# ModelCloud/GPTQModel

Measured on NVIDIA B200. Metric: W4A16 g128 QuantLinear: decode tok/s + prefill TFLOPS vs HBM/TC roofline, higher is better.
Workload: dtype f16

## Files before the change

gptqmodel_b200/_lib.py:

```python
from __future__ import annotations

import ctypes
import os

_HERE = os.path.dirname(os.path.abspath(__file__))
LIB_PATH = os.path.join(_HERE, "libb2q.so")

ABI_VERSION = 3

_vp, _i, _sz = ctypes.c_void_p, ctypes.c_int, ctypes.c_size_t
SYMBOLS = {
    "b2q_version": (_i, []),
    "b2q_last_error": (ctypes.c_char_p, []),
    "b2q_packed_bytes": (_sz, [_i, _i, _i]),
    "b2q_workspace_bytes": (_sz, [_i, _i, _i, _i]),
    "b2q_mm_workspace_bytes": (_sz, [_i, _i, _i, _i, _i, _i]),
    "b2q_debug_reload_env": (None, []),
    "b2q_prepack": (_i, [_vp, _vp, _vp, _i, _i, _i, _vp]),
    "b2q_mm": (_i, [_vp, _vp, _vp, _vp, _vp, _vp, _vp, _i, _i, _i, _i, _i, _i, _vp, _sz, _vp]),
    "b2q_decode": (_i, [_vp, _vp, _vp, _vp, _vp, _vp, _vp, _i, _i, _i, _i, _i, _i, _i, _i, _vp]),
    "b2q_decode_multi": (_i, [_vp, _i, _vp, _vp, _vp, _vp, _vp, _vp, _vp, _i, _i, _i, _i, _i, _vp]),
    "b2q_gemm_multi": (_i, [_vp, _i, _vp, _vp, _vp, _vp, _vp, _vp, _vp, _i, _i, _i, _i, _i, _vp, _sz, _vp]),
    "b2q_gemv": (_i, [_vp, _vp, _vp, _vp, _vp, _vp, _vp, _i, _i, _i, _i, _i, _i, _i, _vp]),
    "b2q_gemm": (_i, [_vp, _vp, _vp, _vp, _vp, _vp, _vp, _i, _i, _i, _i, _i, _i, _vp, _sz, _vp]),
    "b2q_allreduce": (_i, [_vp, _i, _i, _i, _i, _vp, _sz, _i, _vp, _vp]),
    "b2q_decode_allreduce": (_i, [_vp, _vp, _vp, _vp, _vp, _vp, _i, _i, _i, _i, _i, _i, _i, _i, _vp, _sz, _i, _vp, _vp]),
    "b2q_decode_allreduce_flag_bytes": (_sz, []),
    "b2q_debug_set_trace": (None, [_vp]),
    "b2q_debug_decode_plan": (_i, [_i, _i, _i, _i, _i, _i, _vp]),
    "b2q_permute_cols": (_i, [_vp, _vp, _vp, _i, _i, _vp]),
    "b2q_moe_align": (_i, [_vp, _i, _i, _i, _vp, _vp, _vp, _vp]),
    "b2q_moe_gather": (_i, [_vp, _vp, _vp, _i, _i, _i, _vp]),
    "b2q_moe_gate_up": (_i, [_vp, _vp, _vp, _vp, _vp, _vp, _vp, _vp, _vp, _vp, _i, _i, _i, _i, _i, _i, _i, _i, _vp]),
    "b2q_moe_down": (_i, [_vp, _vp, _vp, _vp, _vp, _vp, _vp, _vp, _vp, _i, _i, _i, _i, _i, _i, _i, _i, _vp]),
    "b2q_moe_combine": (_i, [_vp, _vp, _i, _i, _i, _i, _vp]),
    "b2q_moe_decode_gate_up": (_i, [_vp, _vp, _vp, _vp, _vp, _vp, _vp, _vp, _i, _i, _i, _i, _i, _i, _i, _vp, _vp]),
# ... 33 lines not shown
```

gptqmodel_b200/csrc/b2q_api.cu:

```cuda
#include <cstdarg>
#include <cstdio>
#include <cstdlib>

#include "../../include/b2q.h"
#include "b2q_internal.h"

namespace b2q {
static thread_local char g_err[512] = "";

void set_error(const char* fmt, ...) {
  va_list ap;
  va_start(ap, fmt);
  vsnprintf(g_err, sizeof(g_err), fmt, ap);
  va_end(ap);
}

static int env_int(const char* name, int dflt) {
  const char* e = getenv(name);
  return (e != nullptr && e[0] != 0) ? atoi(e) : dflt;
}

static EnvCfg read_env() {
  EnvCfg c;
  c.disable_pdl = env_int("B2Q_DISABLE_PDL", 0);
  c.gemm_1cta = env_int("B2Q_GEMM_1CTA", 0);
  c.midm = env_int("B2Q_MIDM", 1);
  c.decode_blocks_m = env_int("B2Q_DECODE_BLOCKS_M", 0);
  c.decode_groups2 = env_int("B2Q_DECODE_GROUPS", 1) == 2;
  c.decode_v2 = env_int("B2Q_DECODE_V2", -1);
  c.decode2_gw = env_int("B2Q_DECODE2_GW", 0);
  c.decode2_ks = env_int("B2Q_DECODE2_KS", 0);
  c.decode2_xtma = env_int("B2Q_DECODE2_XTMA", 0);
  c.decode2_fastsync = env_int("B2Q_DECODE2_FASTSYNC", 0);
  c.gemm2_persist = env_int("B2Q_GEMM2_PERSIST", 1);
  c.gemm2_dqw = env_int("B2Q_GEMM2_DQW", 8) == 4 ? 4 : 8;
  c.midm_ks = env_int("B2Q_MIDM_KS", 0);
  c.midm_dqg1 = env_int("B2Q_MIDM_DQG1", 0);
  return c;
}

static EnvCfg g_env = read_env();
const EnvCfg& env() { return g_env; }
void reload_env() { g_env = read_env(); }

struct DeviceGuard {
  int prev = -1, dev = -1;
  explicit DeviceGuard(const void* p) {
    cudaPointerAttributes at;
    if (p != nullptr && cudaPointerGetAttributes(&at, p) == cudaSuccess && at.type == cudaMemoryTypeDevice) {
      dev = at.device;
      if (cudaGetDevice(&prev) == cudaSuccess && prev != dev) cudaSetDevice(dev);
      else prev = -1;
    }
    (void)cudaGetLastError();
  }
  ~DeviceGuard() {
    if (prev >= 0) cudaSetDevice(prev);
  }
};

static int check_cuda(int e, const char* what) {
  if (e > 0) set_error("%s: CUDA error %d (%s)", what, e, cudaGetErrorString((cudaError_t)e));
  return e;
}

static int validate(const char* fn, const void* x, const void* packed, const void* scales, const void* out, int M,
                    int K, int N, int bits, int group_size, int dtype) {
  if (x == nullptr || packed == nullptr || scales == nullptr || out == nullptr) {
    set_error("%s: null pointer argument", fn);
    return -2;
  }
  if (bits != 4 && bits != 8) {
    set_error("%s: bits=%d not supported (4 or 8)", fn, bits);
    return -2;
  }
  if (dtype != B2Q_DTYPE_F16 && dtype != B2Q_DTYPE_BF16) {
    set_error("%s: dtype=%d not supported (0 fp16, 1 bf16)", fn, dtype);
    return -2;
// ... 25 lines not shown
  a.perm = perm;
  a.bias = bias;
  a.out = out;
  a.M = M;
  a.K = K;
  a.N = N;
  a.bits = bits;
  a.group_size = group_size;
  a.dtype = dtype;
  a.workspace = workspace;
  a.workspace_bytes = workspace_bytes;
  a.stream = (cudaStream_t)stream;
  a.tune_ks = 0;
  a.tune_warps = 0;
  a.pdl = env().disable_pdl ? 0 : 1;
  return a;
}
}

using namespace b2q;

extern "C" {

int b2q_version(void) { return B2Q_ABI_VERSION; }

void b2q_debug_set_trace(void* device_buffer) { g_trace_ptr = device_buffer; }

int b2q_debug_decode_plan(int version, int M, int K, int N, int ks, int warps, int* out8) {
  if (out8 == nullptr || (version != 1 && version != 2) || M < 1 || M > 8 || K < 128 || K % 128 != 0 || N < 32 ||
      N % 32 != 0) {
// ... 155 lines not shown
  MmArgs a = make_args(x, packed, scales, qzeros, perm, bias, out, M, K, N, bits, group_size, dtype, nullptr, 0,
                       stream);
  a.tune_ks = ks;
  a.tune_warps = warps;
  if (!decode_supported(a)) {
    set_error("b2q_decode: needs bits=4, 1 <= M <= 8, K %% 128 == 0, group_size 64|128|K (got bits=%d M=%d K=%d g=%d)",
              bits, M, K, group_size);
    return -2;
  }
  return check_cuda(launch_decode(a), "b2q_decode");
}

int b2q_decode_multi(const void* x, int nsets, const void* const* packed, const void* const* scales,
                     const int32_t* const* qzeros, const int32_t* perm, const void* const* bias, void* const* out,
                     const int* N, int M, int K, int bits, int group_size, int dtype, void* stream) {
  if (x == nullptr || packed == nullptr || scales == nullptr || qzeros == nullptr || bias == nullptr ||
      out == nullptr || N == nullptr || nsets < 1) {
    set_error("b2q_decode_multi: null pointer argument");
    return -2;
  }
  int v = validate("b2q_decode_multi", x, packed[0], scales[0], out[0], M, K, N[0], bits, group_size, dtype);
  if (v != 0) return v;
  DeviceGuard dg(packed[0]);
  MmArgs a = make_args(x, packed[0], scales[0], qzeros[0], perm, bias[0], out[0], M, K, N[0], bits, group_size,
                       dtype, nullptr, 0, stream);
  return check_cuda(launch_decode_multi(a, nsets, packed, scales, qzeros, bias, out, N), "b2q_decode_multi");
}

int b2q_gemm_multi(const void* x, int nsets, const void* const* packed, const void* const* scales,
                   const int32_t* const* qzeros, const int32_t* perm, const void* const* bias, void* const* out,
                   const int* N, int M, int K, int bits, int group_size, int dtype, void* workspace,
                   size_t workspace_bytes, void* stream) {
  if (x == nullptr || packed == nullptr || scales == nullptr || qzeros == nullptr || bias == nullptr ||
      out == nullptr || N == nullptr || nsets < 1) {
    set_error("b2q_gemm_multi: null pointer argument");
    return -2;
  }
  int v = validate("b2q_gemm_multi", x, packed[0], scales[0], out[0], M, K, N[0], bits, group_size, dtype);
  if (v != 0) return v;
  if (bits != 4 || M <= 128) {
// ... 21 lines not shown
             const void* bias, void* out, int M, int K, int N, int bits, int group_size, int dtype, void* workspace,
             size_t workspace_bytes, void* stream) {
  int v = validate("b2q_gemm", x, packed, scales, out, M, K, N, bits, group_size, dtype);
  if (v != 0) return v;
  DeviceGuard dg(packed);
  if (M == 0) return 0;
  MmArgs a = make_args(x, packed, scales, qzeros, perm, bias, out, M, K, N, bits, group_size, dtype, workspace,
                       workspace_bytes, stream);
  if (env().gemm_1cta) a.tune_ks = -1;
  return check_cuda(launch_gemm(a), "b2q_gemm");
}

int b2q_mm(const void* x, const void* packed, const void* scales, const int32_t* qzeros, const int32_t* perm,
           const void* bias, void* out, int M, int K, int N, int bits, int group_size, int dtype, void* workspace,
           size_t workspace_bytes, void* stream) {
  int v = validate("b2q_mm", x, packed, scales, out, M, K, N, bits, group_size, dtype);
  if (v != 0) return v;
  DeviceGuard dg(packed);
  if (M == 0) return 0;
  MmArgs a = make_args(x, packed, scales, qzeros, perm, bias, out, M, K, N, bits, group_size, dtype, workspace,
                       workspace_bytes, stream);
  if (decode_supported(a)) return check_cuda(launch_decode(a), "b2q_mm(decode)");
  {
    MmArgs a8 = a;
    a8.M = 8;
    if (M > 8 && M <= env().decode_blocks_m && decode_supported(a8) && perm == nullptr) {
      for (int m0 = 0; m0 < M; m0 += 8) {
        MmArgs ab = a;
        ab.M = (M - m0 < 8) ? (M - m0) : 8;
        ab.x = static_cast<const char*>(x) + (size_t)m0 * K * 2;
        ab.out = static_cast<char*>(out) + (size_t)m0 * N * 2;
        int e = check_cuda(launch_decode(ab), "b2q_mm(decode x blocks)");
        if (e != 0) return e;
      }
      return 0;
    }
  }
// ... 141 lines not shown
```

gptqmodel_b200/csrc/b2q_decode.cu:

```cuda
#include "b2q_common.cuh"
#include "b2q_decode.cuh"
#include "b2q_internal.h"

namespace b2q {

template <typename T, bool ASYM, bool G64, bool MOE>
__global__ void __launch_bounds__(DEC_MAX_WARPS * 32)
    decode_kernel(const __grid_constant__ DecSets S, const int32_t* __restrict__ perm, const T* __restrict__ x, int M,
                  int K, int gsh, int qpc, int max_tiles, int ngroups, int stl,
                  const __grid_constant__ DecodeAR ar, unsigned long long* __restrict__ trace) {
  using E = ET<T>;
  extern __shared__ __align__(128) uint8_t dsm[];
  auto stamp = [&](int slot) {
    if (trace != nullptr && threadIdx.x == 0 && blockIdx.y == 0) {
      unsigned long long tns;
      asm volatile("mov.u64 %0, %%globaltimer;" : "=l"(tns));
      trace[blockIdx.x * 16 + slot] = tns;
    }
  };
  stamp(0);
  if (MOE) asm volatile("griddepcontrol.wait;" ::: "memory");
  const int lane = threadIdx.x & 31, warp = threadIdx.x >> 5, nwarps = blockDim.x >> 5;
  const int g = lane >> 2, t = lane & 3;
  const int gw = nwarps / ngroups;
  const int grp = warp / gw, wg = warp - grp * gw;
// ... 32 lines not shown
      iss_q = 0;
      ++iss_ti;
      if (iss_u < U) iss_begin_tile();
    } else {
      iss_src += (size_t)(2 * gw) * iss_kbs;
    }
  };
  if (lane == 0) {
#pragma unroll
    for (int i = 0; i < DEC_STAGES; ++i) mbar_init(bars + 8 * i, 1);
    fence_mbar_init();
    if (U > 0) iss_begin_tile();
#pragma unroll
    for (int i = 0; i < DEC_STAGES; ++i)
      if (i < nst && iss_u < U) iss_one(smem_u32(ring) + i * DEC_QUAD_BYTES, bars + 8 * i);
  }
  const int gstep = (2 * gw) >> gsh;
  const int g_first = (2 * (q0 + wg)) >> gsh;
  const T* sc_next = nullptr;
  const uint32_t* zq_next = nullptr;
  int pre_q = 0, pre_ti = 0, pre_N = 0;
  auto pre_begin_tile = [&]() {
    const TileRef<T> r = resolve_tile<T, MOE>(S, tile0 + pre_ti * C);
    pre_N = r.N;
    sc_next = r.sc + (size_t)g_first * r.N + r.nt * 32 + g;
    if (ASYM) zq_next = r.zq + (size_t)g_first * (r.N >> 3) + r.nt * 4;
  };
  auto fetch_scales = [&](DScale<ASYM, G64>& d) {
#pragma unroll
    for (int i = 0; i < 4; ++i) {
// ... 157 lines not shown
              zh = (float)((cur.zw[ASYM ? gi : 0][ftl * 2 + 1] >> (4 * g)) & 15u);
            }
            const float bl = E::LO_BASE + zl, bh = E::HI_BASE + zh;
            float d[4];
#pragma unroll
            for (int c = 0; c < 4; ++c) d[c] = G64 ? dd[kbl][ftl][c] : dd[0][ftl][c] + dd[1][ftl][c];
            tot[ftl][0] = fmaf(sl, d[0] - bl * xs0, tot[ftl][0]);
            tot[ftl][1] = fmaf(sl, d[1] - bl * xs1, tot[ftl][1]);
            tot[ftl][2] = fmaf(sh, d[2] * E::HI_SCALE - bh * xs0, tot[ftl][2]);
            tot[ftl][3] = fmaf(sh, d[3] * E::HI_SCALE - bh * xs1, tot[ftl][3]);
          }
          xs0 = xs1 = 0.f;
        }
      }
      __syncwarp();
      if (lane == 0 && iss_u < U) iss_one(ring_a + st * DEC_QUAD_BYTES, bars + 8 * st);
      if (u + 1 < U) cur = nxt;
    }

    if (ti < 5) stamp(4 + 2 * ti);
    float* rbuf = red + (grp * 2 + (ti & 1)) * gw * 256;
#pragma unroll
    for (int a = 0; a < 2; ++a)
#pragma unroll
      for (int b = 0; b < 4; ++b) rbuf[(wg * 8 + a * 4 + b) * 32 + lane] = tot[a][b];
    asm volatile("bar.sync %0, %1;" ::"r"(1 + grp), "r"(gw * 32) : "memory");
    for (int i = wg * 32 + lane; i < 256; i += gw * 32) {
      float v = 0.f;
      for (int w = 0; w < gw; ++w) v += rbuf[w * 256 + i];
      if (nrank > 1) {
        part[(grp * max_tiles + ti) * 256 + i] = v;
// ... 76 lines not shown
            if (MOE && S.moe >= 2) pr = S.wts[r] * E::to_f(E::from_f(pr));
            v += pr;
          }
          const int n = nt * 32 + (acc >> 2) * 16 + (ln >> 2) + ((acc & 2) ? 8 : 0);
          T o = E::from_f(v);
          if (bias != nullptr) o = E::from_f(E::to_f(o) + E::to_f(bias[n]));
          out[(size_t)m * N + n] = o;
        }
      }
    }
    cluster_sync_all();
  }
}

void* g_trace_ptr = nullptr;

struct DecodeCfg {
  int C, ks, warps, qpc, max_tiles, ngroups, stl;
  size_t smem;
};

static size_t decode_smem(int M, int warps, int qpc, int max_tiles, int nst) {
  return (size_t)warps * nst * DEC_QUAD_BYTES + (size_t)M * qpc * 128 * 2 + (size_t)qpc * 2 * 8 * 4 +
         (size_t)2 * warps * 256 * 4 + (size_t)max_tiles * 256 * 4 + (size_t)warps * DEC_STAGES * 8 + 16;
}

static bool decode_config(const MmArgs& a, int NT, DecodeCfg& best) {
  const int quads = a.K / 128;
  const int SMS = 148;
  double best_cost = 1e30;
// ... 55 lines not shown
  cfg.blockDim = dim3(c.warps * 32, 1, 1);
  cfg.dynamicSmemBytes = c.smem;
  cfg.stream = a.stream;
  cudaLaunchAttribute attr[2];
  attr[0].id = cudaLaunchAttributeClusterDimension;
  attr[0].val.clusterDim.x = 1;
  attr[0].val.clusterDim.y = c.ks;
  attr[0].val.clusterDim.z = 1;
  attr[1].id = cudaLaunchAttributeProgrammaticStreamSerialization;
  attr[1].val.programmaticStreamSerializationAllowed = 1;
  cfg.attrs = attr;
  cfg.numAttrs = a.pdl ? 2 : 1;
  int gsh = 31;
  if (a.group_size == 64) gsh = 0;
  else if (a.group_size == 128) gsh = 1;
  cudaError_t e = cudaLaunchKernelEx(&cfg, kern, sets, a.perm, (const T*)a.x, a.M, a.K, gsh, c.qpc, c.max_tiles,
                                     c.ngroups, c.stl, ar, (unsigned long long*)g_trace_ptr);
  return (int)e;
}

bool decode_supported(const MmArgs& a) {
  return a.bits == 4 && a.M >= 1 && a.M <= DEC_MAXM && a.K % 128 == 0 && a.N % 32 == 0 &&
         (a.group_size == 64 || a.group_size == 128 || a.group_size == a.K);
}

int launch_decode2_sets(const MmArgs& a, const DecSets& sets);

static int launch_decode_sets(const MmArgs& a, const DecSets& sets) {
  {
    const int mode = env().decode_v2;
    const int NT = sets.tile_end[sets.nsets - 1];
    if (mode == 1 || (mode < 0 && NT > 148 && a.tune_ks <= 0 && a.tune_warps <= 0)) {
// ... 187 lines not shown
```

gptqmodel_b200/csrc/b2q_decode.cuh:

```cuda
#pragma once
#include "b2q_common.cuh"

namespace b2q {

constexpr int DEC_MAX_WARPS = 16;
constexpr int DEC_MAXM = 8;

template <typename T>
__device__ __forceinline__ void mma_16816(float (&d)[4], const uint32_t (&a)[4], uint32_t b0, uint32_t b1);
template <>
__device__ __forceinline__ void mma_16816<__half>(float (&d)[4], const uint32_t (&a)[4], uint32_t b0, uint32_t b1) {
  asm volatile("mma.sync.aligned.m16n8k16.row.col.f32.f16.f16.f32 {%0,%1,%2,%3}, {%4,%5,%6,%7}, {%8,%9}, {%0,%1,%2,%3};"
               : "+f"(d[0]), "+f"(d[1]), "+f"(d[2]), "+f"(d[3])
               : "r"(a[0]), "r"(a[1]), "r"(a[2]), "r"(a[3]), "r"(b0), "r"(b1));
}
template <>
__device__ __forceinline__ void mma_16816<__nv_bfloat16>(float (&d)[4], const uint32_t (&a)[4], uint32_t b0,
                                                         uint32_t b1) {
  asm volatile(
      "mma.sync.aligned.m16n8k16.row.col.f32.bf16.bf16.f32 {%0,%1,%2,%3}, {%4,%5,%6,%7}, {%8,%9}, {%0,%1,%2,%3};"
      : "+f"(d[0]), "+f"(d[1]), "+f"(d[2]), "+f"(d[3])
      : "r"(a[0]), "r"(a[1]), "r"(a[2]), "r"(a[3]), "r"(b0), "r"(b1));
}

// ... 180 lines not shown
  int nsets;
  int tile_end[DEC_MAX_SETS];
  int N[DEC_MAX_SETS];
  const uint4* packed[DEC_MAX_SETS];
  const void* scales[DEC_MAX_SETS];
  const uint32_t* qzeros[DEC_MAX_SETS];
  const void* bias[DEC_MAX_SETS];
  void* out[DEC_MAX_SETS];
  int moe;
  int nexperts;
  const int32_t* ids;
  const float* wts;
  size_t estride_w, estride_s, estride_z;
};

template <typename T>
struct TileRef {
  const uint4* w;
  const T* sc;
  const uint32_t* zq;
  const T* bias;
  T* out;
  int N, nt;
};

template <typename T, bool MOE = false>
__device__ __forceinline__ TileRef<T> resolve_tile(const DecSets& S, int gt) {
  TileRef<T> r;
  if (MOE) {
    int s = 0, nt = gt, slot;
// ... 41 lines not shown
```

gptqmodel_b200/csrc/b2q_decode2.cu:

```cuda
#include "b2q_common.cuh"
#include "b2q_decode.cuh"
#include "b2q_internal.h"

namespace b2q {

constexpr int DEC_AR_MAXCTA = 160;
int launch_decode1_allreduce(const MmArgs& a, const DecSets& sets, const DecodeAR& ar);

__device__ __forceinline__ void cluster_sync_cta_fenced() {
  asm volatile("fence.acq_rel.cta;\n\tbarrier.cluster.arrive.relaxed.aligned;\n\tbarrier.cluster.wait.aligned;" ::: "memory");
}

__device__ __forceinline__ void dec_st_release_sys(uint32_t* p, uint32_t v) {
  asm volatile("st.release.sys.global.u32 [%0], %1;" ::"l"(p), "r"(v) : "memory");
}
__device__ __forceinline__ uint32_t dec_ld_acquire_sys(const uint32_t* p) {
  uint32_t v;
  asm volatile("ld.acquire.sys.global.u32 %0, [%1];" : "=r"(v) : "l"(p) : "memory");
  return v;
}

template <typename T, bool ASYM, bool G64, bool MOE>
__global__ void __launch_bounds__(DEC_MAX_WARPS * 32)
    decode2_kernel(const __grid_constant__ DecSets S, const int32_t* __restrict__ perm, const T* __restrict__ x, int M,
                   int K, int gsh, int qpc, int max_tiles, int gw, int stl, int xtma,
                   const __grid_constant__ DecodeAR ar, unsigned long long* __restrict__ trace) {
  using E = ET<T>;
  extern __shared__ __align__(128) uint8_t dsm2[];
  auto stamp = [&](int slot) {
    if (trace != nullptr && threadIdx.x == 0 && blockIdx.y == 0) {
      unsigned long long tns;
      asm volatile("mov.u64 %0, %%globaltimer;" : "=l"(tns));
      trace[blockIdx.x * 16 + slot] = tns;
    }
  };
  stamp(0);
  if (MOE) asm volatile("griddepcontrol.wait;" ::: "memory");
  const int lane = threadIdx.x & 31, warp = threadIdx.x >> 5, nwarps = blockDim.x >> 5;
  const int g = lane >> 2, t = lane & 3;
  const int ngroups = nwarps / gw;
  const int grp = warp / gw, wg = warp - grp * gw;
// ... 37 lines not shown
      ++iss_ti;
      if (iss_u < U) iss_begin_tile();
    } else {
      iss_src += (size_t)(2 * gw) * iss_kbs;
    }
  };
  if (lane == 0) {
#pragma unroll
    for (int i = 0; i < DEC_STAGES; ++i) mbar_init(bars + 8 * i, 1);
    if (warp == 0) mbar_init(xbar, 1);
    fence_mbar_init();
    if (U > 0) iss_begin_tile();
#pragma unroll
    for (int i = 0; i < DEC_STAGES; ++i)
      if (i < nst && iss_u < U) iss_one(smem_u32(ring) + i * DEC_QUAD_BYTES, bars + 8 * i);
  }
  const int gstep = (2 * gw) >> gsh;
  const int g_first = (2 * (q0 + wg)) >> gsh;
  const T* sc_next = nullptr;
  const uint32_t* zq_next = nullptr;
  int pre_q = 0, pre_ti = 0, pre_N = 0;
  auto pre_begin_tile = [&]() {
    const TileRef<T> r = resolve_tile<T, MOE>(S, tile0 + pre_ti * C);
    pre_N = r.N;
    sc_next = r.sc + (size_t)g_first * r.N + r.nt * 32 + g;
    if (ASYM) zq_next = r.zq + (size_t)g_first * (r.N >> 3) + r.nt * 4;
  };
  auto fetch_scales = [&](DScale<ASYM, G64>& d) {
#pragma unroll
    for (int i = 0; i < 4; ++i) {
// ... 165 lines not shown
              zh = (float)((cur.zw[ASYM ? gi : 0][ftl * 2 + 1] >> (4 * g)) & 15u);
            }
            const float bl = E::LO_BASE + zl, bh = E::HI_BASE + zh;
            float d[4];
#pragma unroll
            for (int c = 0; c < 4; ++c) d[c] = G64 ? dd[kbl][ftl][c] : dd[0][ftl][c] + dd[1][ftl][c];
            tot[ftl][0] = fmaf(sl, d[0] - bl * xs0, tot[ftl][0]);
            tot[ftl][1] = fmaf(sl, d[1] - bl * xs1, tot[ftl][1]);
            tot[ftl][2] = fmaf(sh, d[2] * E::HI_SCALE - bh * xs0, tot[ftl][2]);
            tot[ftl][3] = fmaf(sh, d[3] * E::HI_SCALE - bh * xs1, tot[ftl][3]);
          }
          xs0 = xs1 = 0.f;
        }
      }
      __syncwarp();
      if (lane == 0 && iss_u < U) iss_one(ring_a + st * DEC_QUAD_BYTES, bars + 8 * st);
      if (u + 1 < U) cur = nxt;
    }

    float* wp = wpart + ((size_t)(grp * max_tiles + ti) * M * gw + wg) * 32;
#pragma unroll
    for (int a = 0; a < 2; ++a)
#pragma unroll
      for (int b = 0; b < 4; ++b) {
        const int m = 2 * t + (b & 1);
        if (m < M) {
          const int f = a * 16 + g + ((b & 2) ? 8 : 0);
          wp[(size_t)m * gw * 32 + ((f + 8 * t) & 31)] = tot[a][b];
        }
      }
  }
// ... 173 lines not shown
  cfg.dynamicSmemBytes = c.smem;
  cfg.stream = a.stream;
  cudaLaunchAttribute attr[2];
  attr[0].id = cudaLaunchAttributeClusterDimension;
  attr[0].val.clusterDim.x = 1;
  attr[0].val.clusterDim.y = c.ks;
  attr[0].val.clusterDim.z = 1;
  attr[1].id = cudaLaunchAttributeProgrammaticStreamSerialization;
  attr[1].val.programmaticStreamSerializationAllowed = 1;
  cfg.attrs = attr;
  cfg.numAttrs = a.pdl ? 2 : 1;
  int gsh = 31;
  if (a.group_size == 64) gsh = 0;
  else if (a.group_size == 128) gsh = 1;
  const int xtma = (env().decode2_xtma ? 1 : 0) | (env().decode2_fastsync ? 2 : 0);
  cudaError_t e = cudaLaunchKernelEx(&cfg, kern, sets, a.perm, (const T*)a.x, a.M, a.K, gsh, c.qpc, c.max_tiles, c.gw,
                                     c.stl, xtma, ar, (unsigned long long*)g_trace_ptr);
  return (int)e;
}

static int launch_decode2_ar(const MmArgs& a, const DecSets& sets, const DecodeAR& ar) {
  Decode2Cfg c;
  if (!decode2_config(a, sets.tile_end[sets.nsets - 1], c)) return -2;
  if (ar.world > 1 && c.C * c.ks > DEC_AR_MAXCTA) return -2;
  const bool asym = a.qzeros != nullptr, g64 = a.group_size == 64;
#define B2Q_DEC2_CASE(T, MOE)                                                          \
  (asym ? (g64 ? launch_decode2_t<T, true, true, MOE>(a, sets, c, ar)                      \
               : launch_decode2_t<T, true, false, MOE>(a, sets, c, ar))                    \
        : (g64 ? launch_decode2_t<T, false, true, MOE>(a, sets, c, ar)                     \
               : launch_decode2_t<T, false, false, MOE>(a, sets, c, ar)))
  if (sets.moe != 0) return a.dtype == 0 ? B2Q_DEC2_CASE(__half, true) : B2Q_DEC2_CASE(__nv_bfloat16, true);
  return a.dtype == 0 ? B2Q_DEC2_CASE(__half, false) : B2Q_DEC2_CASE(__nv_bfloat16, false);
// ... 35 lines not shown
```

gptqmodel_b200/csrc/b2q_internal.h:

```cpp
#pragma once
#include <cuda_runtime.h>
#include <stdint.h>

namespace b2q {

struct MmArgs {
  const void* x;
  const void* packed;
  const void* scales;
  const void* qzeros;
  const int32_t* perm;
  const void* bias;
  void* out;
  int M, K, N;
  int bits;
  int group_size;
  int dtype;
  void* workspace;
  size_t workspace_bytes;
  cudaStream_t stream;
  int tune_ks;
  int tune_warps;
  int pdl;
};

struct DecodeAR {
  int world, rank;
  int max_elems;
  size_t flag_offset;
  void* buf[8];
  uint32_t* ctl;
};
int launch_decode_allreduce(const MmArgs& a, const DecodeAR& ar);
size_t decode_allreduce_flag_bytes();

int launch_prepack(const void* qweight, const int32_t* perm, void* out, int K, int N, int bits, cudaStream_t stream);
int launch_permute_cols(const void* x, const int32_t* perm, void* out, int M, int K, cudaStream_t stream);
int launch_gemv(const MmArgs& a);
// ... 39 lines not shown
struct EnvCfg {
  int disable_pdl;
  int gemm_1cta;
  int midm;
  int decode_blocks_m;
  int decode_groups2;
  int decode_v2;
  int decode2_gw;
  int decode2_ks;
  int decode2_xtma;
  int decode2_fastsync;
  int gemm2_persist;
  int gemm2_dqw;
  int midm_ks;
  int midm_dqg1;
};
const EnvCfg& env();
void reload_env();

template <typename Kern>
inline int ensure_dyn_smem(Kern kern, int bytes, uint32_t& done_mask, const char* who) {
  int dev = 0;
  cudaGetDevice(&dev);
  if (dev < 32 && ((done_mask >> dev) & 1u)) return 0;
  cudaError_t e = cudaFuncSetAttribute(kern, cudaFuncAttributeMaxDynamicSharedMemorySize, bytes);
  if (e != cudaSuccess) {
    set_error("%s: cannot opt in to %d bytes of shared memory: %s", who, bytes, cudaGetErrorString(e));
    return (int)e;
  }
  if (dev < 32) done_mask |= 1u << dev;
// ... 6 lines not shown
```

gptqmodel_b200/qlinear.py:

```python
from __future__ import annotations

import os

import math
from typing import Optional, Tuple

import torch
import torch.nn as nn

import ctypes

from . import layouts
from ._lib import B2QError, check, lib
from .adapter import Lora

_DTYPE_CODE = {torch.float16: 0, torch.bfloat16: 1}
DECODE_MAX_M = 8
PREFILL_MIN_M = 128


class SiblingGroup:

    def __init__(self, members):
        self.members = list(members)
        self.key = None
        self.pending = {}
        self._x_ref = None

    @staticmethod
    def _version(t):
        try:
            return t._version
        except RuntimeError:
# ... 8 lines not shown
                self._x_ref = None
            return out
        mods = self.members
        n = len(mods)
        K = who.in_features
        outs = [torch.empty((M, m.out_features), dtype=x2.dtype, device=x2.device) for m in mods]
        vp = ctypes.c_void_p * n
        packed = vp(*[m.packed.data_ptr() for m in mods])
        scales = vp(*[m._scales_for(x2.dtype).data_ptr() for m in mods])
        zeros = vp(*[_ptr(m._zeros_dev) for m in mods])
        bias = vp(*[_ptr(m._bias_for(x2.dtype)) for m in mods])
        outp = vp(*[o.data_ptr() for o in outs])
        Ns = (ctypes.c_int * n)(*[m.out_features for m in mods])
        stream = torch.cuda.current_stream(x2.device).cuda_stream
        if M <= DECODE_MAX_M:
            check(lib.b2q_decode_multi(x2.data_ptr(), n, packed, scales, zeros, _ptr(who.perm), bias, outp, Ns, M, K,
                                       who.kbits, who._kgs, _DTYPE_CODE[x2.dtype], stream), "b2q_decode_multi")
        else:
            ws, ws_bytes = None, 0
            if who.perm is not None:
                ws_bytes = M * K * 2
                ws = torch.empty(ws_bytes, dtype=torch.uint8, device=x2.device)
            check(lib.b2q_gemm_multi(x2.data_ptr(), n, packed, scales, zeros, _ptr(who.perm), bias, outp, Ns, M, K,
                                     who.kbits, who._kgs, _DTYPE_CODE[x2.dtype], _ptr(ws), ws_bytes, stream),
                  "b2q_gemm_multi")
        self.key = key
        self._x_ref = x2
        self.pending = {id(m): o for m, o in zip(mods, outs) if m is not who}
        return outs[mods.index(who)]


def fuse_siblings(mods) -> bool:
# ... 229 lines not shown
            x2 = x2.contiguous()
        M = x2.shape[0]
        if self._siblings is not None and (1 <= M <= DECODE_MAX_M or M > PREFILL_MIN_M):
            return self._siblings.run(self, x2, M).reshape(out_shape)
        out = torch.empty((M, N), dtype=x.dtype, device=x.device)
        if M == 0:
            return out.reshape(out_shape)
        if self._gather is not None:
            x2 = x2.index_select(1, self._gather)
        kK = self._kK
        ws, ws_bytes = None, 0
        if self.perm is not None:
            ws_bytes = lib.b2q_mm_workspace_bytes(M, kK, N, self.kbits, self._kgs, 1)
            if ws_bytes:
                ws = torch.empty(ws_bytes, dtype=torch.uint8, device=x.device)
        check(
            lib.b2q_mm(_ptr(x2), _ptr(self.packed), _ptr(self._scales_for(x.dtype)), _ptr(self._zeros_dev),
                       _ptr(self.perm), _ptr(self._bias_for(x.dtype)), _ptr(out), M, kK, N, self.kbits,
                       self._kgs, _DTYPE_CODE[x.dtype], _ptr(ws), ws_bytes,
                       torch.cuda.current_stream(x.device).cuda_stream),
            "b2q_mm",
        )
        out = out.reshape(out_shape)
        if self.adapter:
            out = self.adapter.apply(x=x, out=out)
        return out

    def forward_allreduce(self, x: torch.Tensor, ar) -> torch.Tensor:
        if not self._prepacked:
            raise B2QError("B200QuantLinear.forward_allreduce() before post_init()")
        K, N = self.in_features, self.out_features
        x2 = x.reshape(-1, K)
        if not x2.is_contiguous():
            x2 = x2.contiguous()
        M = x2.shape[0]
# ... 144 lines not shown
```

include/b2q.h:

```cpp
#ifndef B2Q_H_
#define B2Q_H_

#include <stddef.h>
#include <stdint.h>

#ifdef __cplusplus
extern "C" {
#endif

#define B2Q_ABI_VERSION 3
#define B2Q_DTYPE_F16 0
#define B2Q_DTYPE_BF16 1

int b2q_version(void);

const char* b2q_last_error(void);

size_t b2q_packed_bytes(int K, int N, int bits);

size_t b2q_workspace_bytes(int M, int K, int N, int has_perm);
size_t b2q_mm_workspace_bytes(int M, int K, int N, int bits, int group_size, int has_perm);

int b2q_prepack(const int32_t* qweight, const int32_t* perm, void* packed, int K, int N, int bits, void* stream);

int b2q_mm(const void* x, const void* packed, const void* scales, const int32_t* qzeros, const int32_t* perm,
           const void* bias, void* out, int M, int K, int N, int bits, int group_size, int dtype, void* workspace,
           size_t workspace_bytes, void* stream);

int b2q_decode(const void* x, const void* packed, const void* scales, const int32_t* qzeros, const int32_t* perm,
               const void* bias, void* out, int M, int K, int N, int bits, int group_size, int dtype, int ks,
               int warps, void* stream);
int b2q_gemv(const void* x, const void* packed, const void* scales, const int32_t* qzeros, const int32_t* perm,
             const void* bias, void* out, int K, int N, int bits, int group_size, int dtype, int ks, int warps,
             void* stream);
int b2q_gemm(const void* x, const void* packed, const void* scales, const int32_t* qzeros, const int32_t* perm,
             const void* bias, void* out, int M, int K, int N, int bits, int group_size, int dtype, void* workspace,
             size_t workspace_bytes, void* stream);

int b2q_decode_multi(const void* x, int nsets, const void* const* packed, const void* const* scales,
                     const int32_t* const* qzeros, const int32_t* perm, const void* const* bias, void* const* out,
                     const int* N, int M, int K, int bits, int group_size, int dtype, void* stream);

int b2q_gemm_multi(const void* x, int nsets, const void* const* packed, const void* const* scales,
                   const int32_t* const* qzeros, const int32_t* perm, const void* const* bias, void* const* out,
                   const int* N, int M, int K, int bits, int group_size, int dtype, void* workspace,
                   size_t workspace_bytes, void* stream);

int b2q_moe_align(const int32_t* topk_ids, int T, int top_k, int E, int32_t* counts, int32_t* offsets,
                  int32_t* sorted_pairs, void* stream);
int b2q_moe_gather(const void* x, const int32_t* sorted_pairs, void* xs, int rows, int top_k, int K, void* stream);
int b2q_moe_gate_up(const void* xs, const void* packed1, const void* scales1, const int32_t* qzeros1,
                    const void* packed3, const void* scales3, const int32_t* qzeros3, void* h, const int32_t* counts,
                    const int32_t* offsets, int E, int rows, int active, int K, int N, int bits, int group_size, int dtype,
                    void* stream);
int b2q_moe_down(const void* h, const void* packed2, const void* scales2, const int32_t* qzeros2, const int32_t* counts,
                 const int32_t* offsets, const int32_t* sorted_pairs, const float* pair_weights, float* ypair, int E,
// ... 33 lines not shown
```

Baseline: 866.9.

## Prefetch successor layer's weights into L2 during decode kernel tail

Records the order in which decode launchers run and passes a hint describing the next layer's packed weights, scales, zeros and perm into the decode kernel. Once a CTA has issued its last weight load, its warps issue cp.async.bulk.prefetch.L2 for the first tiles of the successor layer, capped by a configurable byte budget. The aim is to hide the next kernel's cold HBM ramp-up behind the current kernel's tail. In exchange it adds extra HBM traffic that competes with the current kernel's bandwidth, can pull in data that is never used if the recorded successor is wrong, and changes the ABI.

```diff
diff --git a/gptqmodel_b200/_lib.py b/gptqmodel_b200/_lib.py
--- a/gptqmodel_b200/_lib.py
+++ b/gptqmodel_b200/_lib.py
@@ -6,9 +6,24 @@
 _HERE = os.path.dirname(os.path.abspath(__file__))
 LIB_PATH = os.path.join(_HERE, "libb2q.so")
 
-ABI_VERSION = 3
+ABI_VERSION = 4
+
+HINT_MAX_SETS = 3
+
+
+class PrefetchHint(ctypes.Structure):
+    _fields_ = [
+        ("nsets", ctypes.c_int), ("K", ctypes.c_int), ("group_size", ctypes.c_int),
+        ("N", ctypes.c_int * HINT_MAX_SETS),
+        ("packed", ctypes.c_void_p * HINT_MAX_SETS),
+        ("scales", ctypes.c_void_p * HINT_MAX_SETS),
+        ("qzeros", ctypes.c_void_p * HINT_MAX_SETS),
+        ("perm", ctypes.c_void_p),
+    ]
+
 
 _vp, _i, _sz = ctypes.c_void_p, ctypes.c_int, ctypes.c_size_t
+_hint = ctypes.POINTER(PrefetchHint)
 SYMBOLS = {
     "b2q_version": (_i, []),
     "b2q_last_error": (ctypes.c_char_p, []),
@@ -20,6 +35,8 @@
     "b2q_mm": (_i, [_vp, _vp, _vp, _vp, _vp, _vp, _vp, _i, _i, _i, _i, _i, _i, _vp, _sz, _vp]),
     "b2q_decode": (_i, [_vp, _vp, _vp, _vp, _vp, _vp, _vp, _i, _i, _i, _i, _i, _i, _i, _i, _vp]),
     "b2q_decode_multi": (_i, [_vp, _i, _vp, _vp, _vp, _vp, _vp, _vp, _vp, _i, _i, _i, _i, _i, _vp]),
+    "b2q_mm_hinted": (_i, [_vp, _vp, _vp, _vp, _vp, _vp, _vp, _i, _i, _i, _i, _i, _i, _vp, _sz, _vp, _hint]),
+    "b2q_decode_multi_hinted": (_i, [_vp, _i, _vp, _vp, _vp, _vp, _vp, _vp, _vp, _i, _i, _i, _i, _i, _vp, _hint]),
     "b2q_gemm_multi": (_i, [_vp, _i, _vp, _vp, _vp, _vp, _vp, _vp, _vp, _i, _i, _i, _i, _i, _vp, _sz, _vp]),
     "b2q_gemv": (_i, [_vp, _vp, _vp, _vp, _vp, _vp, _vp, _i, _i, _i, _i, _i, _i, _i, _vp]),
     "b2q_gemm": (_i, [_vp, _vp, _vp, _vp, _vp, _vp, _vp, _i, _i, _i, _i, _i, _i, _vp, _sz, _vp]),
diff --git a/gptqmodel_b200/csrc/b2q_api.cu b/gptqmodel_b200/csrc/b2q_api.cu
--- a/gptqmodel_b200/csrc/b2q_api.cu
+++ b/gptqmodel_b200/csrc/b2q_api.cu
@@ -36,6 +36,7 @@
   c.gemm2_dqw = env_int("B2Q_GEMM2_DQW", 8) == 4 ? 4 : 8;
   c.midm_ks = env_int("B2Q_MIDM_KS", 0);
   c.midm_dqg1 = env_int("B2Q_MIDM_DQG1", 0);
+  c.xprefetch_bytes = env_int("B2Q_XPREFETCH_BYTES", 8 << 20);
   return c;
 }
 
@@ -62,6 +63,19 @@
 static int check_cuda(int e, const char* what) {
   if (e > 0) set_error("%s: CUDA error %d (%s)", what, e, cudaGetErrorString((cudaError_t)e));
   return e;
+}
+
+static int validate_hint(const char* fn, const b2q_prefetch_hint* h) {
+  if (h == nullptr || h->nsets == 0) return 0;
+  bool ok = h->nsets > 0 && h->nsets <= B2Q_HINT_MAX_SETS && h->K > 0 && h->K % 64 == 0 && h->group_size > 0 &&
+            h->K % h->group_size == 0;
+  for (int i = 0; ok && i < h->nsets; ++i)
+    ok = h->packed[i] != nullptr && h->scales[i] != nullptr && h->N[i] > 0 && h->N[i] % 32 == 0;
+  if (!ok) {
+    set_error("%s: malformed prefetch hint (nsets=%d K=%d group_size=%d)", fn, h->nsets, h->K, h->group_size);
+    return -2;
+  }
+  return 0;
 }
 
 static int validate(const char* fn, const void* x, const void* packed, const void* scales, const void* out, int M,
@@ -117,6 +131,7 @@
   a.tune_ks = 0;
   a.tune_warps = 0;
   a.pdl = env().disable_pdl ? 0 : 1;
+  a.hint = nullptr;
   return a;
 }
 }
@@ -302,16 +317,26 @@
 int b2q_decode_multi(const void* x, int nsets, const void* const* packed, const void* const* scales,
                      const int32_t* const* qzeros, const int32_t* perm, const void* const* bias, void* const* out,
                      const int* N, int M, int K, int bits, int group_size, int dtype, void* stream) {
+  return b2q_decode_multi_hinted(x, nsets, packed, scales, qzeros, perm, bias, out, N, M, K, bits, group_size, dtype,
+                                 stream, nullptr);
+}
+
+int b2q_decode_multi_hinted(const void* x, int nsets, const void* const* packed, const void* const* scales,
+                            const int32_t* const* qzeros, const int32_t* perm, const void* const* bias, void* const* out,
+                            const int* N, int M, int K, int bits, int group_size, int dtype, void* stream,
+                            const b2q_prefetch_hint* hint) {
   if (x == nullptr || packed == nullptr || scales == nullptr || qzeros == nullptr || bias == nullptr ||
       out == nullptr || N == nullptr || nsets < 1) {
     set_error("b2q_decode_multi: null pointer argument");
     return -2;
   }
   int v = validate("b2q_decode_multi", x, packed[0], scales[0], out[0], M, K, N[0], bits, group_size, dtype);
+  if (v == 0) v = validate_hint("b2q_decode_multi", hint);
   if (v != 0) return v;
   DeviceGuard dg(packed[0]);
   MmArgs a = make_args(x, packed[0], scales[0], qzeros[0], perm, bias[0], out[0], M, K, N[0], bits, group_size,
                        dtype, nullptr, 0, stream);
+  a.hint = hint;
   return check_cuda(launch_decode_multi(a, nsets, packed, scales, qzeros, bias, out, N), "b2q_decode_multi");
 }
 
@@ -363,13 +388,24 @@
 int b2q_mm(const void* x, const void* packed, const void* scales, const int32_t* qzeros, const int32_t* perm,
            const void* bias, void* out, int M, int K, int N, int bits, int group_size, int dtype, void* workspace,
            size_t workspace_bytes, void* stream) {
+  return b2q_mm_hinted(x, packed, scales, qzeros, perm, bias, out, M, K, N, bits, group_size, dtype, workspace,
+                       workspace_bytes, stream, nullptr);
+}
+
+int b2q_mm_hinted(const void* x, const void* packed, const void* scales, const int32_t* qzeros, const int32_t* perm,
+                  const void* bias, void* out, int M, int K, int N, int bits, int group_size, int dtype, void* workspace,
+                  size_t workspace_bytes, void* stream, const b2q_prefetch_hint* hint) {
   int v = validate("b2q_mm", x, packed, scales, out, M, K, N, bits, group_size, dtype);
+  if (v == 0) v = validate_hint("b2q_mm", hint);
   if (v != 0) return v;
   DeviceGuard dg(packed);
   if (M == 0) return 0;
   MmArgs a = make_args(x, packed, scales, qzeros, perm, bias, out, M, K, N, bits, group_size, dtype, workspace,
                        workspace_bytes, stream);
-  if (decode_supported(a)) return check_cuda(launch_decode(a), "b2q_mm(decode)");
+  if (decode_supported(a)) {
+    a.hint = hint;
+    return check_cuda(launch_decode(a), "b2q_mm(decode)");
+  }
   {
     MmArgs a8 = a;
     a8.M = 8;
diff --git a/gptqmodel_b200/csrc/b2q_decode.cu b/gptqmodel_b200/csrc/b2q_decode.cu
--- a/gptqmodel_b200/csrc/b2q_decode.cu
+++ b/gptqmodel_b200/csrc/b2q_decode.cu
@@ -1,3 +1,4 @@
+#include "../../include/b2q.h"
 #include "b2q_common.cuh"
 #include "b2q_decode.cuh"
 #include "b2q_internal.h"
@@ -8,7 +9,8 @@
 __global__ void __launch_bounds__(DEC_MAX_WARPS * 32)
     decode_kernel(const __grid_constant__ DecSets S, const int32_t* __restrict__ perm, const T* __restrict__ x, int M,
                   int K, int gsh, int qpc, int max_tiles, int ngroups, int stl,
-                  const __grid_constant__ DecodeAR ar, unsigned long long* __restrict__ trace) {
+                  const __grid_constant__ DecodeAR ar, const __grid_constant__ DecPrefetch pf,
+                  unsigned long long* __restrict__ trace) {
   using E = ET<T>;
   extern __shared__ __align__(128) uint8_t dsm[];
   auto stamp = [&](int slot) {
@@ -71,6 +73,7 @@
 #pragma unroll
     for (int i = 0; i < DEC_STAGES; ++i)
       if (i < nst && iss_u < U) iss_one(smem_u32(ring) + i * DEC_QUAD_BYTES, bars + 8 * i);
+    if (!MOE && iss_u == U) issue_successor_prefetch(pf);
   }
   const int gstep = (2 * gw) >> gsh;
   const int g_first = (2 * (q0 + wg)) >> gsh;
@@ -258,7 +261,10 @@
         }
       }
       __syncwarp();
-      if (lane == 0 && iss_u < U) iss_one(ring_a + st * DEC_QUAD_BYTES, bars + 8 * st);
+      if (lane == 0 && iss_u < U) {
+        iss_one(ring_a + st * DEC_QUAD_BYTES, bars + 8 * st);
+        if (!MOE && iss_u == U) issue_successor_prefetch(pf);
+      }
       if (u + 1 < U) cur = nxt;
     }
 
@@ -365,6 +371,42 @@
 }
 
 void* g_trace_ptr = nullptr;
+
+DecPrefetch successor_prefetch(const MmArgs& a) {
+  DecPrefetch p = {};
+  const b2q_prefetch_hint* h = a.hint;
+  const long long budget = env().xprefetch_bytes;
+  if (h == nullptr || h->nsets <= 0 || budget <= 0) return p;
+  const int K = h->K, G = K / h->group_size;
+  const bool perm = h->perm != nullptr && (reinterpret_cast<uintptr_t>(h->perm) & 15) == 0;
+  auto add = [&](const void* base, size_t stride, uint32_t row_bytes, int rows) {
+    if (base == nullptr || row_bytes == 0 || rows <= 0 || (reinterpret_cast<uintptr_t>(base) & 15) || (stride & 15))
+      return;
+    DecPrefetch::Region& r = p.r[p.nregions++];
+    r.base = static_cast<const uint8_t*>(base);
+    r.stride = stride;
+    r.row_bytes = row_bytes;
+    r.rows = rows;
+    r.cpr = (int)((row_bytes + DEC_PF_CHUNK - 1) / DEC_PF_CHUNK);
+    r.first = p.chunks;
+    p.chunks += rows * r.cpr;
+  };
+  const long long tile_bytes = (long long)(K / 64) * 1024 + (long long)G * 64 + (h->qzeros[0] != nullptr ? G * 16 : 0);
+  int NT = 0;
+  for (int i = 0; i < h->nsets; ++i) NT += h->N[i] / 32;
+  long long t = NT < 148 ? NT : 148;
+  const long long left = budget - (perm ? (long long)K * 4 : 0);
+  if (t > left / tile_bytes) t = left / tile_bytes;
+  if (perm) add(h->perm + K, (size_t)K * 4, (uint32_t)K * 4, 1);
+  for (int i = 0, start = 0; i < h->nsets && start < t; start += h->N[i] / 32, ++i) {
+    const int ti = (int)(t - start < h->N[i] / 32 ? t - start : h->N[i] / 32);
+    const size_t N = (size_t)h->N[i];
+    add(h->packed[i], N * 32, (uint32_t)ti * 1024, K / 64);
+    add(h->scales[i], N * 2, (uint32_t)ti * 64, G);
+    add(h->qzeros[i], N / 2, (uint32_t)ti * 16, G);
+  }
+  return p;
+}
 
 struct DecodeCfg {
   int C, ks, warps, qpc, max_tiles, ngroups, stl;
@@ -450,8 +492,9 @@
   int gsh = 31;
   if (a.group_size == 64) gsh = 0;
   else if (a.group_size == 128) gsh = 1;
+  const DecPrefetch pf = successor_prefetch(a);
   cudaError_t e = cudaLaunchKernelEx(&cfg, kern, sets, a.perm, (const T*)a.x, a.M, a.K, gsh, c.qpc, c.max_tiles,
-                                     c.ngroups, c.stl, ar, (unsigned long long*)g_trace_ptr);
+                                     c.ngroups, c.stl, ar, pf, (unsigned long long*)g_trace_ptr);
   return (int)e;
 }
 
diff --git a/gptqmodel_b200/csrc/b2q_decode.cuh b/gptqmodel_b200/csrc/b2q_decode.cuh
--- a/gptqmodel_b200/csrc/b2q_decode.cuh
+++ b/gptqmodel_b200/csrc/b2q_decode.cuh
@@ -1,5 +1,6 @@
 #pragma once
 #include "b2q_common.cuh"
+#include "b2q_internal.h"
 
 namespace b2q {
 
@@ -218,6 +219,37 @@
   size_t estride_w, estride_s, estride_z;
 };
 
+constexpr int DEC_PF_MAX = 3 * DEC_MAX_SETS + 1;
+constexpr uint32_t DEC_PF_CHUNK = 8192;
+struct DecPrefetch {
+  int nregions;
+  int chunks;
+  struct Region {
+    const uint8_t* base;
+    size_t stride;
+    uint32_t row_bytes;
+    int rows, cpr;
+    int first;
+  } r[DEC_PF_MAX];
+};
+
+DecPrefetch successor_prefetch(const MmArgs& a);
+
+__device__ __forceinline__ void issue_successor_prefetch(const DecPrefetch& P) {
+  const int nw = blockDim.x >> 5;
+  const int step = gridDim.x * gridDim.y * nw;
+  int ri = 0;
+  for (int j = (int)((blockIdx.y * gridDim.x + blockIdx.x) * nw) + (int)(threadIdx.x >> 5); j < P.chunks; j += step) {
+    while (j >= P.r[ri].first + P.r[ri].rows * P.r[ri].cpr) ++ri;
+    const int local = j - P.r[ri].first;
+    const int row = local / P.r[ri].cpr;
+    const uint32_t off = (uint32_t)(local - row * P.r[ri].cpr) * DEC_PF_CHUNK;
+    const uint32_t bytes = min(DEC_PF_CHUNK, P.r[ri].row_bytes - off);
+    asm volatile("cp.async.bulk.prefetch.L2.global [%0], %1;" ::"l"(P.r[ri].base + (size_t)row * P.r[ri].stride + off),
+                 "r"(bytes) : "memory");
+  }
+}
+
 template <typename T>
 struct TileRef {
   const uint4* w;
diff --git a/gptqmodel_b200/csrc/b2q_decode2.cu b/gptqmodel_b200/csrc/b2q_decode2.cu
--- a/gptqmodel_b200/csrc/b2q_decode2.cu
+++ b/gptqmodel_b200/csrc/b2q_decode2.cu
@@ -24,7 +24,8 @@
 __global__ void __launch_bounds__(DEC_MAX_WARPS * 32)
     decode2_kernel(const __grid_constant__ DecSets S, const int32_t* __restrict__ perm, const T* __restrict__ x, int M,
                    int K, int gsh, int qpc, int max_tiles, int gw, int stl, int xtma,
-                   const __grid_constant__ DecodeAR ar, unsigned long long* __restrict__ trace) {
+                   const __grid_constant__ DecodeAR ar, const __grid_constant__ DecPrefetch pf,
+                  unsigned long long* __restrict__ trace) {
   using E = ET<T>;
   extern __shared__ __align__(128) uint8_t dsm2[];
   auto stamp = [&](int slot) {
@@ -92,6 +93,7 @@
 #pragma unroll
     for (int i = 0; i < DEC_STAGES; ++i)
       if (i < nst && iss_u < U) iss_one(smem_u32(ring) + i * DEC_QUAD_BYTES, bars + 8 * i);
+    if (!MOE && iss_u == U) issue_successor_prefetch(pf);
   }
   const int gstep = (2 * gw) >> gsh;
   const int g_first = (2 * (q0 + wg)) >> gsh;
@@ -287,7 +289,10 @@
         }
       }
       __syncwarp();
-      if (lane == 0 && iss_u < U) iss_one(ring_a + st * DEC_QUAD_BYTES, bars + 8 * st);
+      if (lane == 0 && iss_u < U) {
+        iss_one(ring_a + st * DEC_QUAD_BYTES, bars + 8 * st);
+        if (!MOE && iss_u == U) issue_successor_prefetch(pf);
+      }
       if (u + 1 < U) cur = nxt;
     }
 
@@ -491,8 +496,9 @@
   if (a.group_size == 64) gsh = 0;
   else if (a.group_size == 128) gsh = 1;
   const int xtma = (env().decode2_xtma ? 1 : 0) | (env().decode2_fastsync ? 2 : 0);
+  const DecPrefetch pf = successor_prefetch(a);
   cudaError_t e = cudaLaunchKernelEx(&cfg, kern, sets, a.perm, (const T*)a.x, a.M, a.K, gsh, c.qpc, c.max_tiles, c.gw,
-                                     c.stl, xtma, ar, (unsigned long long*)g_trace_ptr);
+                                     c.stl, xtma, ar, pf, (unsigned long long*)g_trace_ptr);
   return (int)e;
 }
 
diff --git a/gptqmodel_b200/csrc/b2q_internal.h b/gptqmodel_b200/csrc/b2q_internal.h
--- a/gptqmodel_b200/csrc/b2q_internal.h
+++ b/gptqmodel_b200/csrc/b2q_internal.h
@@ -1,6 +1,8 @@
 #pragma once
 #include <cuda_runtime.h>
 #include <stdint.h>
+
+struct b2q_prefetch_hint;
 
 namespace b2q {
 
@@ -22,6 +24,7 @@
   int tune_ks;
   int tune_warps;
   int pdl;
+  const b2q_prefetch_hint* hint;
 };
 
 struct DecodeAR {
@@ -91,6 +94,7 @@
   int gemm2_dqw;
   int midm_ks;
   int midm_dqg1;
+  int xprefetch_bytes;
 };
 const EnvCfg& env();
 void reload_env();
diff --git a/gptqmodel_b200/qlinear.py b/gptqmodel_b200/qlinear.py
--- a/gptqmodel_b200/qlinear.py
+++ b/gptqmodel_b200/qlinear.py
@@ -3,6 +3,7 @@
 import os
 
 import math
+import weakref
 from typing import Optional, Tuple
 
 import torch
@@ -11,12 +12,74 @@
 import ctypes
 
 from . import layouts
-from ._lib import B2QError, check, lib
+from ._lib import HINT_MAX_SETS, B2QError, PrefetchHint, check, lib
 from .adapter import Lora
 
 _DTYPE_CODE = {torch.float16: 0, torch.bfloat16: 1}
 DECODE_MAX_M = 8
 PREFILL_MIN_M = 128
+
+
+class LaunchChain:
+
+    def __init__(self):
+        self._last = None
+        self._next = weakref.WeakKeyDictionary()
+
+    def record(self, launcher):
+        prev = self._last() if self._last is not None else None
+        if prev is not None and prev is not launcher:
+            self._next[prev] = weakref.ref(launcher)
+        self._last = weakref.ref(launcher)
+
+    def successor(self, launcher):
+        r = self._next.get(launcher)
+        return r() if r is not None else None
+
+    def reset(self):
+        self._last = None
+        self._next = weakref.WeakKeyDictionary()
+
+
+_CHAINS = {}
+
+
+def launch_chain(device: torch.device) -> LaunchChain:
+    key = device.index if device.index is not None else torch.cuda.current_device()
+    c = _CHAINS.get(key)
+    if c is None:
+        c = _CHAINS[key] = LaunchChain()
+    return c
+
+
+def _decode_sets(launcher):
+    return (launcher.members, launcher.members[0]) if isinstance(launcher, SiblingGroup) else ([launcher], launcher)
+
+
+def prefetch_hint(launcher, device, dtype):
+    succ = launch_chain(device).successor(launcher)
+    if succ is None:
+        launcher._hint_cache = None
+        return None
+    c = getattr(launcher, "_hint_cache", None)
+    if c is not None and c[0]() is succ and c[1] == dtype:
+        return c[2]
+    mods, m0 = _decode_sets(succ)
+    h = PrefetchHint()
+    h.nsets, h.K, h.group_size = len(mods), m0._kK, m0._kgs
+    for i, m in enumerate(mods[:HINT_MAX_SETS]):
+        h.N[i] = m.out_features
+        h.packed[i] = m.packed.data_ptr()
+        h.scales[i] = m._scales_for(dtype).data_ptr()
+        h.qzeros[i] = _ptr(m._zeros_dev)
+    h.perm = _ptr(m0.perm)
+    launcher._hint_cache = (weakref.ref(succ), dtype, ctypes.pointer(h))
+    return launcher._hint_cache[2]
+
+
+def _decode_launch_hint(launcher, device, dtype):
+    launch_chain(device).record(launcher)
+    return prefetch_hint(launcher, device, dtype)
 
 
 class SiblingGroup:
@@ -55,8 +118,10 @@
         Ns = (ctypes.c_int * n)(*[m.out_features for m in mods])
         stream = torch.cuda.current_stream(x2.device).cuda_stream
         if M <= DECODE_MAX_M:
-            check(lib.b2q_decode_multi(x2.data_ptr(), n, packed, scales, zeros, _ptr(who.perm), bias, outp, Ns, M, K,
-                                       who.kbits, who._kgs, _DTYPE_CODE[x2.dtype], stream), "b2q_decode_multi")
+            hint = _decode_launch_hint(self, x2.device, x2.dtype)
+            check(lib.b2q_decode_multi_hinted(x2.data_ptr(), n, packed, scales, zeros, _ptr(who.perm), bias, outp, Ns, M,
+                                              K, who.kbits, who._kgs, _DTYPE_CODE[x2.dtype], stream, hint),
+                  "b2q_decode_multi")
         else:
             ws, ws_bytes = None, 0
             if who.perm is not None:
@@ -316,11 +381,14 @@
             ws_bytes = lib.b2q_mm_workspace_bytes(M, kK, N, self.kbits, self._kgs, 1)
             if ws_bytes:
                 ws = torch.empty(ws_bytes, dtype=torch.uint8, device=x.device)
+        hint = None
+        if M <= DECODE_MAX_M and self.kbits == 4 and kK % 128 == 0 and self._kgs in (64, 128, kK):
+            hint = _decode_launch_hint(self, x.device, x.dtype)
         check(
-            lib.b2q_mm(_ptr(x2), _ptr(self.packed), _ptr(self._scales_for(x.dtype)), _ptr(self._zeros_dev),
-                       _ptr(self.perm), _ptr(self._bias_for(x.dtype)), _ptr(out), M, kK, N, self.kbits,
-                       self._kgs, _DTYPE_CODE[x.dtype], _ptr(ws), ws_bytes,
-                       torch.cuda.current_stream(x.device).cuda_stream),
+            lib.b2q_mm_hinted(_ptr(x2), _ptr(self.packed), _ptr(self._scales_for(x.dtype)), _ptr(self._zeros_dev),
+                              _ptr(self.perm), _ptr(self._bias_for(x.dtype)), _ptr(out), M, kK, N, self.kbits,
+                              self._kgs, _DTYPE_CODE[x.dtype], _ptr(ws), ws_bytes,
+                              torch.cuda.current_stream(x.device).cuda_stream, hint),
             "b2q_mm",
         )
         out = out.reshape(out_shape)
diff --git a/include/b2q.h b/include/b2q.h
--- a/include/b2q.h
+++ b/include/b2q.h
@@ -8,7 +8,7 @@
 extern "C" {
 #endif
 
-#define B2Q_ABI_VERSION 3
+#define B2Q_ABI_VERSION 4
 #define B2Q_DTYPE_F16 0
 #define B2Q_DTYPE_BF16 1
 
@@ -37,9 +37,28 @@
              const void* bias, void* out, int M, int K, int N, int bits, int group_size, int dtype, void* workspace,
              size_t workspace_bytes, void* stream);
 
+#define B2Q_HINT_MAX_SETS 3
+typedef struct b2q_prefetch_hint {
+  int nsets;
+  int K, group_size;
+  int N[B2Q_HINT_MAX_SETS];
+  const void* packed[B2Q_HINT_MAX_SETS];
+  const void* scales[B2Q_HINT_MAX_SETS];
+  const int32_t* qzeros[B2Q_HINT_MAX_SETS];
+  const int32_t* perm;
+} b2q_prefetch_hint;
+
+int b2q_mm_hinted(const void* x, const void* packed, const void* scales, const int32_t* qzeros, const int32_t* perm,
+                  const void* bias, void* out, int M, int K, int N, int bits, int group_size, int dtype, void* workspace,
+                  size_t workspace_bytes, void* stream, const b2q_prefetch_hint* hint);
+
 int b2q_decode_multi(const void* x, int nsets, const void* const* packed, const void* const* scales,
                      const int32_t* const* qzeros, const int32_t* perm, const void* const* bias, void* const* out,
                      const int* N, int M, int K, int bits, int group_size, int dtype, void* stream);
+int b2q_decode_multi_hinted(const void* x, int nsets, const void* const* packed, const void* const* scales,
+                            const int32_t* const* qzeros, const int32_t* perm, const void* const* bias, void* const* out,
+                            const int* N, int M, int K, int bits, int group_size, int dtype, void* stream,
+                            const b2q_prefetch_hint* hint);
 
 int b2q_gemm_multi(const void* x, int nsets, const void* const* packed, const void* const* scales,
                    const int32_t* const* qzeros, const int32_t* perm, const void* const* bias, void* const* out,
```

Measured after the change: 845.3, median of 6. 0.975x the previous value.
